# ZrrSkywalker/MonoDETR

Measured on NVIDIA H100. Metric: images/sec (1280x384, fwd+bwd), higher is better.
Workload: dtype f32 (BF16x3: error-compensated bf16 tensor-core products, fp32 accumulate)

## Files before the change

### monodetr_b200/csrc/conv_gemm.cu

```cuda
#include <cuda.h>
#include <cuda_runtime.h>
#include <stdint.h>
#include <stdlib.h>
#include <string.h>

#include "../../include/monodetr_b200.h"
#include "launch.cuh"
#include "tc_common.cuh"
#include "tma_host.cuh"

namespace {

using namespace mdb;

constexpr int BM = 128;
constexpr int BK = 32;
constexpr int kTileABytes = BM * 128;
constexpr int kChunkBytes = 32 * 128;
constexpr int kConsumerThreads = 256;
constexpr int kThreadsTC = kConsumerThreads + 32;
constexpr int kMaxTaps = 9;

struct TcParams {
    int tiles_x, tiles_y, tw, th, tb;
    int Ho, Wo;
    int out_sy, out_sx, out_oy, out_ox, out_H, out_W;
    int in_sy, in_sx;
    int ntaps, cblocks;
    int tap_dy[kMaxTaps], tap_dx[kMaxTaps], tap_w[kMaxTaps];
    int rtiles_x, rtiles_y, rtw, rth, n_img, red_per_split;
    int kb_per_slice, slice_stride;
    int total_tiles, n_tiles_n, n_tiles_m;
    int w_sy, w_sx, wg_taps, wg_kw, wg_pad;
    int Mo_rows;
    int No, ldo;
    int relu, atomic_out, round_out;
    int epi_tma, epi_load, half_x, half_y, half_b;
    const float* bias;
    const float* residual;
    const float* relu_mask;
    const float* rowscale;
    float* out;
};

template <bool MN>
__device__ __forceinline__ uint32_t raw_off(int row, int k) {
    if constexpr (MN) return (uint32_t)((row >> 5) * kChunkBytes + k * 128 + (((((row & 31) >> 2) ^ (k & 7))) << 4) + (row & 3) * 4);
    else return (uint32_t)(row * 128 + (((k >> 2) ^ (row & 7)) << 4) + (k & 3) * 4);
}

__device__ __forceinline__ float trunc_tf32(float x) { return __uint_as_float(__float_as_uint(x) & 0xFFFFE000u); }

template <int BN, int STAGES, int MODE, int PREC>
struct TcSmem {
    static constexpr bool kConvB = !(PREC == 2 && MODE == 0);
    static constexpr int kRing = STAGES * (kTileABytes + BN * 128);
    static constexpr int kStage = 2 * 64 * BN * 4;
    static constexpr int kConvBuf = kConvB ? (PREC == 1 ? 2 : 1) * BN * 128 : 0;
    static constexpr int kConv = 2 * kConvBuf;
    static constexpr int kFixed = kRing + kConv + 1024  + 256 ;
    static constexpr bool kTmaEpi = MODE == 0 && kFixed + kStage <= 227 * 1024;
    static constexpr int kBytes = kFixed + (kTmaEpi ? kStage : 0);
};

template <int BN, int STAGES, int MODE , bool B_MN, int PREC>
__global__ void __launch_bounds__(kThreadsTC, 1)
tc_conv_gemm_kernel(const __grid_constant__ CUtensorMap mapA, const __grid_constant__ CUtensorMap mapB,
                    const __grid_constant__ CUtensorMap mapO, const __grid_constant__ CUtensorMap mapR,
                    const __grid_constant__ TcParams p) {
    constexpr bool A_MN = (MODE == 1);
    static_assert(!(MODE == 1) || B_MN, "wgrad reads both operands MN-major");
    static_assert(BN == 64 || BN == 128, "tile width");
    constexpr bool BF_B = (PREC == 2 && MODE == 0);
    static_assert(!BF_B || !B_MN, "pre-split weights are K-major");
    constexpr bool CONVB = !BF_B;
    constexpr int kTileBBytes = BN * 128;
    constexpr int kRawBytes = kTileABytes + kTileBBytes;
    using SM = TcSmem<BN, STAGES, MODE, PREC>;
    constexpr int NACC = BN / 2;

    extern __shared__ __align__(1024) uint8_t smem[];
    uint8_t* stage_out = smem + STAGES * kRawBytes;
    uint8_t* bconv = stage_out + (SM::kTmaEpi ? SM::kStage : 0);
    uint64_t* full_bar = reinterpret_cast<uint64_t*>(bconv + SM::kConv);
    uint64_t* empty_bar = full_bar + STAGES;
    uint64_t* epi_bar = empty_bar + STAGES;

    const int warp = threadIdx.x >> 5;
    const int lane = threadIdx.x & 31;

    struct Tile { int n0, img, y0, x0, m0, red_begin, iters, tap, slice; };
    auto decode = [&](int tix) {
        Tile t;
        t.n0 = (tix % p.n_tiles_n) * BN;
        int r = tix / p.n_tiles_n;
        t.img = t.y0 = t.x0 = t.m0 = t.red_begin = t.tap = t.slice = 0;
        if constexpr (MODE == 0) {
            const int per_img = p.tiles_x * p.tiles_y;
            t.iters = p.ntaps * p.cblocks;
            if (p.kb_per_slice > 0) {
                t.slice = r / p.n_tiles_m;
                r -= t.slice * p.n_tiles_m;
                t.red_begin = t.slice * p.kb_per_slice;
                t.iters = max(0, min(t.iters, t.red_begin + p.kb_per_slice) - t.red_begin);
            }
            const int grp = r / per_img;
            t.img = grp * p.tb;
            r -= grp * per_img;
            t.y0 = (r / p.tiles_x) * p.th;
            t.x0 = (r % p.tiles_x) * p.tw;
        } else {
            t.m0 = (r % p.n_tiles_m) * BM;
            r /= p.n_tiles_m;
            t.tap = r % p.wg_taps;
            const int z = r / p.wg_taps;
            const int total_red = p.n_img * p.rtiles_x * p.rtiles_y;
            t.red_begin = z * p.red_per_split;
            t.iters = max(0, min(total_red, t.red_begin + p.red_per_split) - t.red_begin);
        }
        return t;
    };

    if (threadIdx.x == 0) {
        if (smem_u32(smem) & 1023u) __trap();
        tma_prefetch_desc(&mapA);
        tma_prefetch_desc(&mapB);
        if (SM::kTmaEpi && p.epi_tma) {
            tma_prefetch_desc(&mapO);
            if (p.epi_load) tma_prefetch_desc(&mapR);
        }
        for (int s = 0; s < STAGES; ++s) {
            mbar_init(&full_bar[s], 1);
            mbar_init(&empty_bar[s], kConsumerThreads / 32);
        }
        mbar_init(&epi_bar[0], 1);
        mbar_init(&epi_bar[1], 1);
        fence_mbar_init();
    }
    __syncthreads();
    asm volatile("griddepcontrol.wait;" ::: "memory");
    asm volatile("griddepcontrol.launch_dependents;" ::: "memory");

    if (warp == kConsumerThreads / 32) {
        if (elect_one()) {
            int git = 0;
            for (int tix = blockIdx.x; tix < p.total_tiles; tix += gridDim.x) {
                const Tile t = decode(tix);
                for (int it = 0; it < t.iters; ++it, ++git) {
                    const int s = git % STAGES;
                    const uint32_t ph = (git / STAGES) & 1;
                    mbar_wait(&empty_bar[s], ph ^ 1);
                    uint8_t* a_dst = smem + s * kRawBytes;
                    uint8_t* b_dst = a_dst + kTileABytes;
                    mbar_arrive_expect_tx(&full_bar[s], kRawBytes);
                    if constexpr (MODE == 0) {
                        const int kit = t.red_begin + it;
                        const int tap = kit / p.cblocks;
                        const int cb = kit - tap * p.cblocks;
                        tma_load_4d(a_dst, &mapA, &full_bar[s], cb * BK, t.x0 * p.in_sx + p.tap_dx[tap],
                                    t.y0 * p.in_sy + p.tap_dy[tap], t.img);
                        if constexpr (BF_B) {
                            tma_load_3d(b_dst, &mapB, &full_bar[s], cb * 64, t.n0, p.tap_w[tap]);
                        } else if constexpr (!B_MN) {
                            tma_load_3d(b_dst, &mapB, &full_bar[s], cb * BK, t.n0, p.tap_w[tap]);
                        } else {
#pragma unroll
                            for (int j = 0; j < BN / 32; ++j)
                                tma_load_3d(b_dst + j * kChunkBytes, &mapB, &full_bar[s], t.n0 + j * 32, cb * BK, p.tap_w[tap]);
                        }
                    } else {
                        int r = t.red_begin + it;
                        const int per_img = p.rtiles_x * p.rtiles_y;
                        const int ri = r / per_img;
                        r -= ri * per_img;
                        const int ry = (r / p.rtiles_x) * p.rth;
                        const int rx = (r % p.rtiles_x) * p.rtw;
#pragma unroll
                        for (int j = 0; j < BM / 32; ++j)
                            tma_load_4d(a_dst + j * kChunkBytes, &mapA, &full_bar[s], t.m0 + j * 32, rx, ry, ri);
#pragma unroll
                        for (int j = 0; j < BN / 32; ++j)
                            tma_load_4d(b_dst + j * kChunkBytes, &mapB, &full_bar[s], t.n0 + j * 32,
                                        rx * p.w_sx + (t.tap % p.wg_kw) - p.wg_pad, ry * p.w_sy + (t.tap / p.wg_kw) - p.wg_pad, ri);
                    }
                }
            }
        }
        return;
    }
    if (warp > kConsumerThreads / 32) return;

    const int wg = warp >> 2;
    const int g = lane >> 2, tig = lane & 3;
    const int r0 = wg * 64 + (warp & 3) * 16 + g;
    const int ctid = threadIdx.x;
    const bool epi_tma = SM::kTmaEpi && p.epi_tma;
    const bool leader = (ctid & 127) == 0;
    uint8_t* my_stage = stage_out + wg * (SM::kStage / 2);
    uint32_t epi_phase = 0;
    constexpr int KS = PREC == 2 ? 2 : 4;
    using Frag = uint32_t[KS][4];
    auto load_kblock = [&](int gi, int buf, Frag& hi, Frag& lo) {
        const int s = gi % STAGES;
        mbar_wait(&full_bar[s], (gi / STAGES) & 1);
        const uint8_t* a_raw = smem + s * kRawBytes;
        if constexpr (CONVB) {
            const uint8_t* b_raw = a_raw + kTileABytes;
            uint8_t* bc = bconv + buf * SM::kConvBuf;
            named_bar_sync(1, kConsumerThreads);
            if constexpr (PREC == 2) {
#pragma unroll
                for (int i = ctid; i < BN * 4; i += kConsumerThreads) {
                    const int n = i % BN, c = i / BN;
                    float x[8];
#pragma unroll
                    for (int e = 0; e < 8; ++e) x[e] = *reinterpret_cast<const float*>(b_raw + raw_off<B_MN>(n, 8 * c + e));
                    uint32_t hw[4], lw[4];
#pragma unroll
                    for (int e = 0; e < 4; ++e) {
                        const uint32_t h = pack_bf16x2(x[2 * e], x[2 * e + 1]);
                        hw[e] = h;
                        lw[e] = pack_bf16x2(x[2 * e] - __uint_as_float(h << 16), x[2 * e + 1] - __uint_as_float(h & 0xFFFF0000u));
                    }
                    uint8_t* brow = bc + n * 128;
                    *reinterpret_cast<uint4*>(brow + ((c ^ (n & 7)) << 4)) = make_uint4(hw[0], hw[1], hw[2], hw[3]);
                    *reinterpret_cast<uint4*>(brow + (((4 + c) ^ (n & 7)) << 4)) = make_uint4(lw[0], lw[1], lw[2], lw[3]);
                }
            } else {
#pragma unroll 4
                for (int i = ctid; i < BN * 8; i += kConsumerThreads) {
                    const int n = i % BN, c = i / BN;
                    float4 x;
                    if constexpr (B_MN) {
                        x.x = *reinterpret_cast<const float*>(b_raw + raw_off<true>(n, 4 * c));
                        x.y = *reinterpret_cast<const float*>(b_raw + raw_off<true>(n, 4 * c + 1));
                        x.z = *reinterpret_cast<const float*>(b_raw + raw_off<true>(n, 4 * c + 2));
                        x.w = *reinterpret_cast<const float*>(b_raw + raw_off<true>(n, 4 * c + 3));
                    } else {
                        x = *reinterpret_cast<const float4*>(b_raw + raw_off<false>(n, 4 * c));
                    }
                    const float4 h = make_float4(trunc_tf32(x.x), trunc_tf32(x.y), trunc_tf32(x.z), trunc_tf32(x.w));
                    const uint32_t off = n * 128 + ((c ^ (n & 7)) << 4);
                    *reinterpret_cast<float4*>(bc + off) = h;
                    if constexpr (PREC == 1)
                        *reinterpret_cast<float4*>(bc + kTileBBytes + off) = make_float4(x.x - h.x, x.y - h.y, x.z - h.z, x.w - h.w);
                }
            }
            fence_proxy_async_smem();
            named_bar_sync(1, kConsumerThreads);
        }
#pragma unroll
        for (int ks = 0; ks < KS; ++ks) {
#pragma unroll
            for (int f = 0; f < 4; ++f) {
                const int row = r0 + (f & 1) * 8;
                if constexpr (PREC == 2) {
                    const int k = ks * 16 + tig * 2 + (f >> 1) * 8;
                    float x0, x1;
                    if constexpr (A_MN) {
                        x0 = *reinterpret_cast<const float*>(a_raw + raw_off<true>(row, k));
                        x1 = *reinterpret_cast<const float*>(a_raw + raw_off<true>(row, k + 1));
                    } else {
                        const float2 v = *reinterpret_cast<const float2*>(a_raw + raw_off<false>(row, k));
                        x0 = v.x; x1 = v.y;
                    }
                    const uint32_t h = pack_bf16x2(x0, x1);
                    hi[ks][f] = h;
                    lo[ks][f] = pack_bf16x2(x0 - __uint_as_float(h << 16), x1 - __uint_as_float(h & 0xFFFF0000u));
                } else {
                    const int k = ks * 8 + tig + (f >> 1) * 4;
                    const float x = *reinterpret_cast<const float*>(a_raw + raw_off<A_MN>(row, k));
                    const float h = trunc_tf32(x);
                    hi[ks][f] = __float_as_uint(h);
                    lo[ks][f] = __float_as_uint(x - h);
                }
            }
        }
    };
    auto issue_kblock = [&](int gi, int buf, const Frag& hi, const Frag& lo, float (&acc)[NACC]) {
        const uint32_t b_addr = smem_u32(CONVB ? bconv + buf * SM::kConvBuf : smem + (gi % STAGES) * kRawBytes + kTileABytes);
        wgmma_fence();
#pragma unroll
        for (int ks = 0; ks < KS; ++ks) {
            const uint64_t bhi = make_wgmma_desc_sw128(b_addr + ks * 32);
            const uint64_t blo = make_wgmma_desc_sw128(b_addr + (PREC == 2 ? 64 : kTileBBytes) + ks * 32);
            if constexpr (PREC == 2) {
                if constexpr (BN == 128) {
                    wgmma_bf16_n128(acc, hi[ks], bhi, 1);
                    wgmma_bf16_n128(acc, lo[ks], bhi, 1);
                    wgmma_bf16_n128(acc, hi[ks], blo, 1);
                } else {
                    wgmma_bf16_n64(acc, hi[ks], bhi, 1);
                    wgmma_bf16_n64(acc, lo[ks], bhi, 1);
                    wgmma_bf16_n64(acc, hi[ks], blo, 1);
                }
            } else {
                if constexpr (BN == 128) wgmma_tf32_n128(acc, hi[ks], bhi, 1);
                else wgmma_tf32_n64(acc, hi[ks], bhi, 1);
                if constexpr (PREC == 1) {
                    if constexpr (BN == 128) {
                        wgmma_tf32_n128(acc, lo[ks], bhi, 1);
                        wgmma_tf32_n128(acc, hi[ks], blo, 1);
                    } else {
                        wgmma_tf32_n64(acc, lo[ks], bhi, 1);
                        wgmma_tf32_n64(acc, hi[ks], blo, 1);
                    }
                }
            }
        }
        wgmma_commit();
    };
    int git = 0;
    for (int tix = blockIdx.x; tix < p.total_tiles; tix += gridDim.x) {
        const Tile t = decode(tix);
        if (p.atomic_out && t.iters == 0) continue;
        const int c1 = t.x0 + wg * p.half_x, c2 = t.y0 + wg * p.half_y, c3 = t.img + wg * p.half_b, c4 = t.slice;
        if (epi_tma && p.epi_load && leader) {
            bulk_wait_read_all();
            mbar_arrive_expect_tx(&epi_bar[wg], SM::kStage / 2);
#pragma unroll
            for (int c = 0; c < BN / 32; ++c) tma_load_5d(my_stage + c * 8192, &mapR, &epi_bar[wg], t.n0 + 32 * c, c1, c2, c3, c4);
        }
        float acc[NACC];
#pragma unroll
        for (int i = 0; i < NACC; ++i) acc[i] = 0.f;
        if (t.iters > 0) {
            Frag ahi0, alo0, ahi1, alo1;
            auto step = [&](int it, const Frag& chi, const Frag& clo, Frag& nhi, Frag& nlo) {
                issue_kblock(git + it, it & 1, chi, clo, acc);
                wgmma_wait<1>();
                wgmma_fence_operands(nhi);
                wgmma_fence_operands(nlo);
                if (it > 0) {
                    __syncwarp();
                    if (lane == 0) mbar_arrive(&empty_bar[(git + it - 1) % STAGES]);
                }
                if (it + 1 < t.iters) load_kblock(git + it + 1, (it + 1) & 1, nhi, nlo);
            };
            load_kblock(git, 0, ahi0, alo0);
            for (int it = 0; it < t.iters; it += 2) {
                step(it, ahi0, alo0, ahi1, alo1);
                if (it + 1 < t.iters) step(it + 1, ahi1, alo1, ahi0, alo0);
            }
            wgmma_wait<0>();
            wgmma_fence_operands(acc);
            wgmma_fence_operands(ahi0);
            wgmma_fence_operands(alo0);
            wgmma_fence_operands(ahi1);
            wgmma_fence_operands(alo1);
            __syncwarp();
            if (lane == 0) mbar_arrive(&empty_bar[(git + t.iters - 1) % STAGES]);
            git += t.iters;
        }

        if (epi_tma) {
            if (p.bias) {
#pragma unroll
                for (int j = 0; j < BN / 8; ++j) {
                    const int n = t.n0 + j * 8 + tig * 2;
                    if (n >= p.No) continue;
                    const float b0 = p.bias[n], b1 = p.bias[n + 1];
                    acc[4 * j] += b0; acc[4 * j + 1] += b1; acc[4 * j + 2] += b0; acc[4 * j + 3] += b1;
                }
            }
            if (p.epi_load) {
                mbar_wait(&epi_bar[wg], epi_phase);
                epi_phase ^= 1;
            } else {
                if (leader) bulk_wait_read_all();
                named_bar_sync(2 + wg, 128);
            }
            constexpr int kMB = 8;
#pragma unroll
            for (int h = 0; h < 2; ++h) {
                const int row = r0 + h * 8, rr = row - 64 * wg;
                const float* gmask = nullptr;
                if (p.relu_mask && p.epi_load != 2) {
                    const int lyt = row / p.tw, lx = row - lyt * p.tw;
                    const int ib = lyt / p.th, ly = lyt - ib * p.th;
                    const int y = t.y0 + ly, x = t.x0 + lx, img = t.img + ib;
                    if ((y < p.Ho) && (x < p.Wo) && (img < p.n_img))
                        gmask = p.relu_mask + (size_t)((img * p.out_H + y * p.out_sy + p.out_oy) * p.out_W + x * p.out_sx + p.out_ox) * p.ldo;
                }
#pragma unroll
                for (int j0 = 0; j0 < BN / 8; j0 += kMB) {
                    float2 mv[kMB];
#pragma unroll
                    for (int u = 0; u < kMB; ++u) {
                        const int n = t.n0 + (j0 + u) * 8 + tig * 2;
                        mv[u] = (gmask && n < p.No) ? *reinterpret_cast<const float2*>(gmask + n) : make_float2(0.f, 0.f);
                    }
#pragma unroll
                    for (int u = 0; u < kMB; ++u) {
                        const int j = j0 + u, n = t.n0 + j * 8 + tig * 2;
                        if (n >= p.No) continue;
                        float2* sp = reinterpret_cast<float2*>(my_stage + (j >> 2) * 8192 + raw_off<false>(rr, (j & 3) * 8 + tig * 2));
                        float v[2] = {acc[4 * j + 2 * h], acc[4 * j + 2 * h + 1]};
                        if (p.epi_load == 1) { const float2 e = *sp; v[0] += e.x; v[1] += e.y; }
                        if (p.relu) { v[0] = fmaxf(v[0], 0.f); v[1] = fmaxf(v[1], 0.f); }
                        if (p.relu_mask) {
                            const float2 m = p.epi_load == 2 ? *sp : mv[u];
                            v[0] = m.x > 0.f ? v[0] : 0.f; v[1] = m.y > 0.f ? v[1] : 0.f;
                        }
                        if (p.round_out) { v[0] = round_tf32(v[0]); v[1] = round_tf32(v[1]); }
                        *sp = make_float2(v[0], v[1]);
                    }
                }
            }
            fence_proxy_async_smem();
            named_bar_sync(2 + wg, 128);
            if (leader) {
#pragma unroll
                for (int c = 0; c < BN / 32; ++c) tma_store_5d(&mapO, my_stage + c * 8192, t.n0 + 32 * c, c1, c2, c3, c4);
                bulk_commit();
            }
            continue;
        }
#pragma unroll
        for (int h = 0; h < 2; ++h) {
            const int row = r0 + h * 8;
            bool ok;
            size_t roff;
            float rsc = 1.f;
            if constexpr (MODE == 0) {
                const int lyt = row / p.tw, lx = row - lyt * p.tw;
                const int ib = lyt / p.th, ly = lyt - ib * p.th;
                const int y = t.y0 + ly, x = t.x0 + lx, img = t.img + ib;
                ok = (y < p.Ho) && (x < p.Wo) && (img < p.n_img);
                const int oy = y * p.out_sy + p.out_oy, ox = x * p.out_sx + p.out_ox;
                roff = (size_t)((img * p.out_H + oy) * p.out_W + ox) * p.ldo + (size_t)t.slice * p.slice_stride;
            } else {
                ok = (t.m0 + row) < p.Mo_rows;
                if (ok && p.rowscale) rsc = p.rowscale[t.m0 + row];
                roff = (size_t)(t.tap * p.Mo_rows + t.m0 + row) * p.ldo;
            }
            if (!ok) continue;
            const bool vec = !(p.ldo & 1);
#pragma unroll
            for (int j = 0; j < BN / 8; ++j) {
                const int n = t.n0 + j * 8 + tig * 2;
                if (n >= p.No) continue;
                float v[2] = {acc[4 * j + 2 * h] * rsc, acc[4 * j + 2 * h + 1] * rsc};
                const bool pair = vec && n + 1 < p.No;
                if (p.bias) { v[0] += p.bias[n]; if (pair) v[1] += p.bias[n + 1]; }
                if (p.residual) {
                    if (pair) { const float2 e = *reinterpret_cast<const float2*>(p.residual + roff + n); v[0] += e.x; v[1] += e.y; }
                    else v[0] += p.residual[roff + n];
                }
                if (p.relu) { v[0] = fmaxf(v[0], 0.f); v[1] = fmaxf(v[1], 0.f); }
                if (p.relu_mask) {
                    if (pair) {
                        const float2 m = *reinterpret_cast<const float2*>(p.relu_mask + roff + n);
                        v[0] = m.x > 0.f ? v[0] : 0.f; v[1] = m.y > 0.f ? v[1] : 0.f;
                    } else {
                        v[0] = p.relu_mask[roff + n] > 0.f ? v[0] : 0.f;
                    }
                }
                if (p.round_out) { v[0] = round_tf32(v[0]); v[1] = round_tf32(v[1]); }
                float* dst = p.out + roff + n;
                if (pair) {
                    if (p.atomic_out) red_add_v2_f32(dst, v[0], v[1]);
                    else *reinterpret_cast<float2*>(dst) = make_float2(v[0], v[1]);
                } else {
                    for (int e = 0; e < 2 && n + e < p.No; ++e) {
                        float x = e == 0 ? v[0] : acc[4 * j + 2 * h + 1] * rsc;
                        if (e == 1) {
                            if (p.bias) x += p.bias[n + 1];
                            if (p.residual) x += p.residual[roff + n + 1];
                            if (p.relu) x = fmaxf(x, 0.f);
                            if (p.relu_mask) x = p.relu_mask[roff + n + 1] > 0.f ? x : 0.f;
                            if (p.round_out) x = round_tf32(x);
                        }
                        if (p.atomic_out) atomicAdd(dst + e, x);
                        else dst[e] = x;
                    }
                }
            }
        }
    }
    if (epi_tma && leader) bulk_wait_all();
}

int g_precision = 2;

constexpr int kMaxDevices = 64;
struct DeviceState {
    float* ws = nullptr;
    size_t ws_bytes = 0;
};
DeviceState g_dev[kMaxDevices];

int current_device() {
    int dev = 0;
    if (cudaGetDevice(&dev) != cudaSuccess || dev < 0 || dev >= kMaxDevices) return 0;
    return dev;
}

template <int BN, int STAGES, int MODE, bool B_MN, int PREC>
int launch_tc(const CUtensorMap& a, const CUtensorMap& b, const CUtensorMap& o, const CUtensorMap& r, TcParams p, dim3 grid,
              cudaStream_t stream) {
    constexpr int smem = TcSmem<BN, STAGES, MODE, PREC>::kBytes;
    static_assert(smem <= 227 * 1024, "dynamic shared memory budget");
    if (!TcSmem<BN, STAGES, MODE, PREC>::kTmaEpi) p.epi_tma = p.epi_load = 0;
    auto kern = tc_conv_gemm_kernel<BN, STAGES, MODE, B_MN, PREC>;
    const cudaError_t e = set_max_dynamic_smem(kern, smem);
    if (e != cudaSuccess) return (int)e;
    p.n_tiles_n = (int)grid.x;
    p.n_tiles_m = (int)grid.y;
    p.total_tiles = (int)(grid.x * grid.y * grid.z);
    int ctas = num_sms();
    if (ctas > p.total_tiles) ctas = p.total_tiles;
    if (ctas < 1) return 0;
    static const bool pdl = getenv("MDB_NO_PDL") == nullptr;
    if (pdl) {
        cudaLaunchConfig_t cfg;
        memset(&cfg, 0, sizeof(cfg));
        cfg.gridDim = dim3((unsigned)ctas, 1, 1);
        cfg.blockDim = dim3((unsigned)kThreadsTC, 1, 1);
        cfg.dynamicSmemBytes = smem;
        cfg.stream = stream;
        cudaLaunchAttribute attr[1];
        attr[0].id = cudaLaunchAttributeProgrammaticStreamSerialization;
        attr[0].val.programmaticStreamSerializationAllowed = 1;
        cfg.attrs = attr;
        cfg.numAttrs = 1;
        return (int)cudaLaunchKernelEx(&cfg, kern, a, b, o, r, p);
    }
    kern<<<ctas, kThreadsTC, smem, stream>>>(a, b, o, r, p);
    return (int)cudaGetLastError();
}

__global__ void splitk_reduce_kernel(const float4* __restrict__ ws, const float4* __restrict__ bias, float4* __restrict__ y,
                                     long long n4, int N4, int slices, long long stride4) {
    for (long long i = blockIdx.x * (long long)blockDim.x + threadIdx.x; i < n4; i += (long long)gridDim.x * blockDim.x) {
        float4 a = bias ? bias[i % N4] : make_float4(0.f, 0.f, 0.f, 0.f);
        for (int z = 0; z < slices; ++z) {
            const float4 v = ws[z * stride4 + i];
            a.x += v.x; a.y += v.y; a.z += v.z; a.w += v.w;
        }
        y[i] = a;
    }
}

int splitk_workspace(size_t bytes, float** out) {
    DeviceState& d = g_dev[current_device()];
    if (bytes > d.ws_bytes || !d.ws) return MDB_EWORKSPACE;
    *out = d.ws;
    return 0;
}

void pick_tile(int W, int H, int n_pix, int* tw, int* th) {
    int best_tw = n_pix, best_waste = 1 << 30;
    for (int w = n_pix; w >= 1; w >>= 1) {
        const int h = n_pix / w;
        const int tx = (W + w - 1) / w, ty = (H + h - 1) / h;
        const int waste = tx * w * ty * h - W * H;
        if (waste < best_waste) { best_waste = waste; best_tw = w; }
    }
    *tw = best_tw;
    *th = n_pix / best_tw;
}

void pick_tile3(int W, int H, int B, int n_pix, int* tw, int* th, int* tb) {
    long long best = -1;
    *tw = n_pix; *th = 1; *tb = 1;
    for (int b = 1; b <= n_pix; b <<= 1)
        for (int w = n_pix / b; w >= 1; w >>= 1) {
            const int h = n_pix / b / w;
            if (b > 1 && b >= 2 * B) continue;
            const long long cov = (long long)((W + w - 1) / w) * w * ((H + h - 1) / h) * h * ((B + b - 1) / b) * b;
            if (best < 0 || cov < best) { best = cov; *tw = w; *th = h; *tb = b; }
        }
}

bool aligned16(const void* q) { return (reinterpret_cast<uintptr_t>(q) & 15u) == 0; }

int setup_epi_px(TcParams& p, CUtensorMap* mo, CUtensorMap* mr, size_t off, int Wc, int Hc, int B, uint64_t sx, uint64_t sy,
                 uint64_t sb, int slices) {
    p.epi_tma = p.epi_load = p.half_x = p.half_y = p.half_b = 0;
    if (p.No % 4 || p.ldo % 4 || !aligned16(p.out + off) || (p.residual && !aligned16(p.residual + off)) ||
        (p.relu_mask && !aligned16(p.relu_mask + off)))
        return 0;
    uint32_t box[5] = {32, (uint32_t)p.tw, (uint32_t)p.th, (uint32_t)p.tb, 1};
    if (p.tb > 1) p.half_b = box[3] = p.tb / 2;
    else if (p.th > 1) p.half_y = box[2] = p.th / 2;
    else p.half_x = box[1] = p.tw / 2;
    if (box[1] > 256 || box[2] > 256 || box[3] > 256) return 0;
    uint64_t dims[5] = {(uint64_t)p.No, (uint64_t)Wc, (uint64_t)Hc, (uint64_t)B, (uint64_t)slices};
    uint64_t str[5] = {1, sx, sy, sb, slices > 1 ? (uint64_t)p.slice_stride : sb * B};
    int rc = make_map(mo, p.out + off, 5, dims, str, box, nullptr);
    if (rc) return rc;
    const float* opnd = p.residual ? p.residual : p.relu_mask;
    if (opnd) {
        rc = make_map(mr, opnd + off, 5, dims, str, box, nullptr);
        if (rc) return rc;
        p.epi_load = p.residual ? 1 : 2;
    }
    p.epi_tma = 1;
    return 0;
}

int launch_fwd(const CUtensorMap& ma, const CUtensorMap& mb, const CUtensorMap& mo, const CUtensorMap& mr, const TcParams& p, dim3 grid, int bn, int precision, cudaStream_t stream) {
    if (precision == 2) return bn == 64 ? launch_tc<64, 6, 0, false, 2>(ma, mb, mo, mr, p, grid, stream) : launch_tc<128, 5, 0, false, 2>(ma, mb, mo, mr, p, grid, stream);
    if (precision == 1) return bn == 64 ? launch_tc<64, 5, 0, false, 1>(ma, mb, mo, mr, p, grid, stream) : launch_tc<128, 3, 0, false, 1>(ma, mb, mo, mr, p, grid, stream);
    return bn == 64 ? launch_tc<64, 6, 0, false, 0>(ma, mb, mo, mr, p, grid, stream) : launch_tc<128, 5, 0, false, 0>(ma, mb, mo, mr, p, grid, stream);
}

struct ConvGeom {
    int B, H, W, Cin, Cout, kh, kw, stride, pad, Ho, Wo;
};

// ... 236 lines not shown
    d.ws = static_cast<float*>(buf);
    d.ws_bytes = buf ? (size_t)bytes : 0;
    return 0;
}
int mdb_conv2d_dgrad_f32(const float* dy, const float* w_packed, const float* residual, const float* relu_mask,
                         float* dx, int B, int H, int W, int Cin, int Cout, int kh, int kw, int stride, int pad,
                         int flags, void* stream) {
    return conv_dgrad_impl(dy, w_packed, false, residual, relu_mask, dx, B, H, W, Cin, Cout, kh, kw, stride, pad, flags, stream);
}
int mdb_conv2d_dgrad_bf16x3(const float* dy, const void* w_split_t, const float* residual, const float* relu_mask,
                            float* dx, int B, int H, int W, int Cin, int Cout, int kh, int kw, int stride, int pad,
                            int flags, void* stream) {
    return conv_dgrad_impl(dy, w_split_t, true, residual, relu_mask, dx, B, H, W, Cin, Cout, kh, kw, stride, pad, flags, stream);
}

int mdb_conv2d_wgrad_f32(const float* dy, const float* x, const float* rowscale, float* dw_packed, int B, int H, int W,
                         int Cin, int Cout, int kh, int kw, int stride, int pad, int accumulate, void* stream_) {
    return mdb_conv2d_wgrad_bias_f32(dy, x, rowscale, dw_packed, nullptr, B, H, W, Cin, Cout, kh, kw, stride, pad, accumulate, stream_);
}

int mdb_conv2d_wgrad_bias_f32(const float* dy, const float* x, const float* rowscale, float* dw_packed, float* db, int B, int H,
                              int W, int Cin, int Cout, int kh, int kw, int stride, int pad, int accumulate, void* stream_) {
    ConvGeom g{B, H, W, Cin, Cout, kh, kw, stride, pad, (H + 2 * pad - kh) / stride + 1, (W + 2 * pad - kw) / stride + 1};
    int rc = check_geom(g);
    if (rc) return rc;
    if (!dy || !x || !dw_packed) return MDB_EINVAL;
    cudaStream_t stream = static_cast<cudaStream_t>(stream_);
    if (kh == 1 && stride == 1 && pad == 0) {
        W = B * H * W; H = 1; B = 1;
        g = ConvGeom{B, H, W, Cin, Cout, kh, kw, stride, pad, H, W};
    }
    const int taps = kh * kw;
    if (!accumulate) {
        cudaError_t e = cudaMemsetAsync(dw_packed, 0, sizeof(float) * (size_t)taps * Cout * Cin, stream);
        if (e != cudaSuccess) return (int)e;
    }
    if (db) {
        rc = mdb_colsum_f32(dy, db, (long long)B * g.Ho * g.Wo, Cout, accumulate, stream_);
        if (rc) return rc;
    }
    TcParams p;
    memset(&p, 0, sizeof(p));
    pick_tile(g.Wo, g.Ho, 32, &p.rtw, &p.rth);
    p.rtiles_x = (g.Wo + p.rtw - 1) / p.rtw;
    p.rtiles_y = (g.Ho + p.rth - 1) / p.rth;
    p.n_img = B;
    const int total_red = B * p.rtiles_x * p.rtiles_y;
    const int bn = 128;
    const int tiles = ((Cout + BM - 1) / BM) * ((Cin + bn - 1) / bn) * taps;
    const int sms = num_sms();
    int big = (2 * sms + tiles - 1) / tiles, small = sms / tiles;
    if (big > total_red / 24) big = total_red / 24;
    if (small > total_red / 8) small = total_red / 8;
    int splits = big > small ? big : small;
    if (splits < 1 || mdb_get_deterministic()) splits = 1;
    p.red_per_split = (total_red + splits - 1) / splits;
    splits = (total_red + p.red_per_split - 1) / p.red_per_split;
    p.w_sy = p.w_sx = stride;
    p.wg_taps = taps; p.wg_kw = kw; p.wg_pad = pad;
    p.Mo_rows = Cout; p.No = Cin; p.ldo = Cin; p.relu = 0; p.atomic_out = 1;
    p.bias = nullptr; p.residual = nullptr; p.relu_mask = nullptr; p.rowscale = rowscale;
    p.out = dw_packed;

    CUtensorMap ma, mb;
    {
        uint64_t dims[4] = {(uint64_t)Cout, (uint64_t)g.Wo, (uint64_t)g.Ho, (uint64_t)B};
        uint64_t str[4] = {1, (uint64_t)Cout, (uint64_t)g.Wo * Cout, (uint64_t)g.Ho * g.Wo * Cout};
        uint32_t box[4] = {32, (uint32_t)p.rtw, (uint32_t)p.rth, 1};
        rc = make_map(&ma, dy, 4, dims, str, box, nullptr);
        if (rc) return rc;
    }
    {
        uint64_t dims[4] = {(uint64_t)Cin, (uint64_t)W, (uint64_t)H, (uint64_t)B};
        uint64_t str[4] = {1, (uint64_t)Cin, (uint64_t)W * Cin, (uint64_t)H * W * Cin};
        uint32_t box[4] = {32, (uint32_t)(p.rtw * stride), (uint32_t)(p.rth * stride), 1};
        uint32_t es[4] = {1, (uint32_t)stride, (uint32_t)stride, 1};
        rc = make_map(&mb, x, 4, dims, str, box, es);
        if (rc) return rc;
    }
    CUtensorMap mo, mr;
    memset(&mo, 0, sizeof(mo));
    memset(&mr, 0, sizeof(mr));
    dim3 grid((Cin + bn - 1) / bn, (Cout + BM - 1) / BM, taps * splits);
    rc = g_precision == 2 ? launch_tc<128, 4, 1, true, 2>(ma, mb, mo, mr, p, grid, stream)
         : g_precision == 1 ? launch_tc<128, 4, 1, true, 1>(ma, mb, mo, mr, p, grid, stream)
                            : launch_tc<128, 5, 1, true, 0>(ma, mb, mo, mr, p, grid, stream);
    if (rc) return rc;
    return 0;
}

}
```

### monodetr_b200/csrc/tc_common.cuh

```cuda
#pragma once
#include <cuda.h>
#include <cuda_runtime.h>
#include <stdint.h>

namespace mdb {

__device__ __forceinline__ uint32_t smem_u32(const void* p) {
    return static_cast<uint32_t>(__cvta_generic_to_shared(p));
}

__device__ __forceinline__ bool elect_one() {
    uint32_t pred = 0;
    asm volatile(
        "{\n\t.reg .b32 rx;\n\t.reg .pred px;\n\t"
        "elect.sync rx|px, 0xffffffff;\n\t"
        "selp.b32 %0, 1, 0, px;\n\t}"
        : "=r"(pred));
    return pred != 0;
}

__device__ __forceinline__ void mbar_init(uint64_t* bar, uint32_t count) {
    asm volatile("mbarrier.init.shared::cta.b64 [%0], %1;" ::"r"(smem_u32(bar)), "r"(count) : "memory");
}
__device__ __forceinline__ void fence_mbar_init() {
// ... 26 lines not shown
    uint32_t spins = 0;
    uint64_t t0 = 0;
    while (!mbar_try_wait(bar, parity)) {
        if (++spins == 16384u) {
            spins = 0;
            mbar_slow_path(t0);
        }
    }
}

__device__ __forceinline__ void fence_proxy_async_smem() { asm volatile("fence.proxy.async.shared::cta;" ::: "memory"); }
__device__ __forceinline__ void named_bar_sync(int id, int count) { asm volatile("bar.sync %0, %1;" ::"r"(id), "r"(count) : "memory"); }

__device__ __forceinline__ void tma_prefetch_desc(const CUtensorMap* m) {
    asm volatile("prefetch.tensormap [%0];" ::"l"(reinterpret_cast<uint64_t>(m)) : "memory");
}
__device__ __forceinline__ void tma_load_2d(void* dst, const CUtensorMap* m, uint64_t* bar, int c0, int c1) {
    asm volatile(
        "cp.async.bulk.tensor.2d.shared::cluster.global.mbarrier::complete_tx::bytes [%0], [%1, {%3, %4}], [%2];" ::"r"(
            smem_u32(dst)),
        "l"(reinterpret_cast<uint64_t>(m)), "r"(smem_u32(bar)), "r"(c0), "r"(c1)
        : "memory");
}
__device__ __forceinline__ void tma_load_3d(void* dst, const CUtensorMap* m, uint64_t* bar, int c0, int c1, int c2) {
    asm volatile(
        "cp.async.bulk.tensor.3d.shared::cluster.global.mbarrier::complete_tx::bytes [%0], [%1, {%3, %4, %5}], [%2];" ::"r"(
            smem_u32(dst)),
        "l"(reinterpret_cast<uint64_t>(m)), "r"(smem_u32(bar)), "r"(c0), "r"(c1), "r"(c2)
        : "memory");
}
__device__ __forceinline__ void tma_load_4d(void* dst, const CUtensorMap* m, uint64_t* bar, int c0, int c1, int c2,
                                            int c3) {
    asm volatile(
        "cp.async.bulk.tensor.4d.shared::cluster.global.mbarrier::complete_tx::bytes [%0], [%1, {%3, %4, %5, %6}], "
        "[%2];" ::"r"(smem_u32(dst)),
        "l"(reinterpret_cast<uint64_t>(m)), "r"(smem_u32(bar)), "r"(c0), "r"(c1), "r"(c2), "r"(c3)
        : "memory");
}
__device__ __forceinline__ void tma_load_5d(void* dst, const CUtensorMap* m, uint64_t* bar, int c0, int c1, int c2,
                                            int c3, int c4) {
    asm volatile(
        "cp.async.bulk.tensor.5d.shared::cluster.global.mbarrier::complete_tx::bytes [%0], [%1, {%3, %4, %5, %6, %7}], "
        "[%2];" ::"r"(smem_u32(dst)),
        "l"(reinterpret_cast<uint64_t>(m)), "r"(smem_u32(bar)), "r"(c0), "r"(c1), "r"(c2), "r"(c3), "r"(c4)
        : "memory");
}
__device__ __forceinline__ void tma_store_5d(const CUtensorMap* m, const void* src, int c0, int c1, int c2, int c3, int c4) {
    asm volatile("cp.async.bulk.tensor.5d.global.shared::cta.bulk_group [%0, {%2, %3, %4, %5, %6}], [%1];"
                 ::"l"(reinterpret_cast<uint64_t>(m)), "r"(smem_u32(src)), "r"(c0), "r"(c1), "r"(c2), "r"(c3), "r"(c4)
                 : "memory");
}
__device__ __forceinline__ void bulk_commit() { asm volatile("cp.async.bulk.commit_group;" ::: "memory"); }
__device__ __forceinline__ void bulk_wait_read_all() { asm volatile("cp.async.bulk.wait_group.read 0;" ::: "memory"); }
__device__ __forceinline__ void bulk_wait_all() { asm volatile("cp.async.bulk.wait_group 0;" ::: "memory"); }

__device__ __forceinline__ void wgmma_fence() { asm volatile("wgmma.fence.sync.aligned;" ::: "memory"); }
__device__ __forceinline__ void wgmma_commit() { asm volatile("wgmma.commit_group.sync.aligned;" ::: "memory"); }
__device__ __forceinline__ void wgmma_wait_all() { asm volatile("wgmma.wait_group.sync.aligned 0;" ::: "memory"); }
template <int N>
__device__ __forceinline__ void wgmma_wait() { asm volatile("wgmma.wait_group.sync.aligned %0;" ::"n"(N) : "memory"); }
template <int N>
__device__ __forceinline__ void wgmma_fence_operands(float (&d)[N]) {
#pragma unroll
    for (int i = 0; i < N; ++i) asm volatile("" : "+f"(d[i])::"memory");
}
template <int M, int N>
__device__ __forceinline__ void wgmma_fence_operands(uint32_t (&a)[M][N]) {
#pragma unroll
    for (int i = 0; i < M; ++i)
#pragma unroll
        for (int j = 0; j < N; ++j) asm volatile("" : "+r"(a[i][j])::"memory");
}
__device__ __forceinline__ void wgmma_bf16_n64(float (&d)[32], const uint32_t (&a)[4], uint64_t bdesc, int scale_d) {
    asm volatile(
        "{\n\t.reg .pred p;\n\t"
        "setp.ne.b32 p, %37, 0;\n\t"
        "wgmma.mma_async.sync.aligned.m64n64k16.f32.bf16.bf16 "
        "{%0, %1, %2, %3, %4, %5, %6, %7, %8, %9, %10, %11, %12, %13, %14, %15, "
        "%16, %17, %18, %19, %20, %21, %22, %23, %24, %25, %26, %27, %28, %29, %30, %31"
        "}, {%32, %33, %34, %35}, %36, p, 1, 1, 0;\n\t}"
        : "+f"(d[0]), "+f"(d[1]), "+f"(d[2]), "+f"(d[3]), "+f"(d[4]), "+f"(d[5]), "+f"(d[6]), "+f"(d[7]), "+f"(d[8]), "+f"(d[9]), "+f"(d[10]), "+f"(d[11]), "+f"(d[12]), "+f"(d[13]), "+f"(d[14]), "+f"(d[15]), "+f"(d[16]), "+f"(d[17]), "+f"(d[18]), "+f"(d[19]), "+f"(d[20]), "+f"(d[21]), "+f"(d[22]), "+f"(d[23]), "+f"(d[24]), "+f"(d[25]), "+f"(d[26]), "+f"(d[27]), "+f"(d[28]), "+f"(d[29]), "+f"(d[30]), "+f"(d[31])
        : "r"(a[0]), "r"(a[1]), "r"(a[2]), "r"(a[3]), "l"(bdesc), "r"(scale_d));
}
__device__ __forceinline__ void wgmma_bf16_n128(float (&d)[64], const uint32_t (&a)[4], uint64_t bdesc, int scale_d) {
    asm volatile(
        "{\n\t.reg .pred p;\n\t"
        "setp.ne.b32 p, %69, 0;\n\t"
        "wgmma.mma_async.sync.aligned.m64n128k16.f32.bf16.bf16 "
        "{%0, %1, %2, %3, %4, %5, %6, %7, %8, %9, %10, %11, %12, %13, %14, %15, "
        "%16, %17, %18, %19, %20, %21, %22, %23, %24, %25, %26, %27, %28, %29, %30, %31, "
        "%32, %33, %34, %35, %36, %37, %38, %39, %40, %41, %42, %43, %44, %45, %46, %47, "
        "%48, %49, %50, %51, %52, %53, %54, %55, %56, %57, %58, %59, %60, %61, %62, %63"
        "}, {%64, %65, %66, %67}, %68, p, 1, 1, 0;\n\t}"
        : "+f"(d[0]), "+f"(d[1]), "+f"(d[2]), "+f"(d[3]), "+f"(d[4]), "+f"(d[5]), "+f"(d[6]), "+f"(d[7]), "+f"(d[8]), "+f"(d[9]), "+f"(d[10]), "+f"(d[11]), "+f"(d[12]), "+f"(d[13]), "+f"(d[14]), "+f"(d[15]), "+f"(d[16]), "+f"(d[17]), "+f"(d[18]), "+f"(d[19]), "+f"(d[20]), "+f"(d[21]), "+f"(d[22]), "+f"(d[23]), "+f"(d[24]), "+f"(d[25]), "+f"(d[26]), "+f"(d[27]), "+f"(d[28]), "+f"(d[29]), "+f"(d[30]), "+f"(d[31]), "+f"(d[32]), "+f"(d[33]), "+f"(d[34]), "+f"(d[35]), "+f"(d[36]), "+f"(d[37]), "+f"(d[38]), "+f"(d[39]), "+f"(d[40]), "+f"(d[41]), "+f"(d[42]), "+f"(d[43]), "+f"(d[44]), "+f"(d[45]), "+f"(d[46]), "+f"(d[47]), "+f"(d[48]), "+f"(d[49]), "+f"(d[50]), "+f"(d[51]), "+f"(d[52]), "+f"(d[53]), "+f"(d[54]), "+f"(d[55]), "+f"(d[56]), "+f"(d[57]), "+f"(d[58]), "+f"(d[59]), "+f"(d[60]), "+f"(d[61]), "+f"(d[62]), "+f"(d[63])
        : "r"(a[0]), "r"(a[1]), "r"(a[2]), "r"(a[3]), "l"(bdesc), "r"(scale_d));
}
__device__ __forceinline__ void wgmma_tf32_n32(float (&d)[16], const uint32_t (&a)[4], uint64_t bdesc, int scale_d) {
    asm volatile(
        "{\n\t.reg .pred p;\n\t"
        "setp.ne.b32 p, %21, 0;\n\t"
        "wgmma.mma_async.sync.aligned.m64n32k8.f32.tf32.tf32 "
        "{%0, %1, %2, %3, %4, %5, %6, %7, %8, %9, %10, %11, %12, %13, %14, %15"
        "}, {%16, %17, %18, %19}, %20, p, 1, 1;\n\t}"
        : "+f"(d[0]), "+f"(d[1]), "+f"(d[2]), "+f"(d[3]), "+f"(d[4]), "+f"(d[5]), "+f"(d[6]), "+f"(d[7]), "+f"(d[8]), "+f"(d[9]), "+f"(d[10]), "+f"(d[11]), "+f"(d[12]), "+f"(d[13]), "+f"(d[14]), "+f"(d[15])
        : "r"(a[0]), "r"(a[1]), "r"(a[2]), "r"(a[3]), "l"(bdesc), "r"(scale_d));
}

__device__ __forceinline__ void wgmma_tf32_n64(float (&d)[32], const uint32_t (&a)[4], uint64_t bdesc, int scale_d) {
    asm volatile(
        "{\n\t.reg .pred p;\n\t"
        "setp.ne.b32 p, %37, 0;\n\t"
        "wgmma.mma_async.sync.aligned.m64n64k8.f32.tf32.tf32 "
        "{%0, %1, %2, %3, %4, %5, %6, %7, %8, %9, %10, %11, %12, %13, %14, %15, "
        "%16, %17, %18, %19, %20, %21, %22, %23, %24, %25, %26, %27, %28, %29, %30, %31"
        "}, {%32, %33, %34, %35}, %36, p, 1, 1;\n\t}"
        : "+f"(d[0]), "+f"(d[1]), "+f"(d[2]), "+f"(d[3]), "+f"(d[4]), "+f"(d[5]), "+f"(d[6]), "+f"(d[7]), "+f"(d[8]), "+f"(d[9]), "+f"(d[10]), "+f"(d[11]), "+f"(d[12]), "+f"(d[13]), "+f"(d[14]), "+f"(d[15]), "+f"(d[16]), "+f"(d[17]), "+f"(d[18]), "+f"(d[19]), "+f"(d[20]), "+f"(d[21]), "+f"(d[22]), "+f"(d[23]), "+f"(d[24]), "+f"(d[25]), "+f"(d[26]), "+f"(d[27]), "+f"(d[28]), "+f"(d[29]), "+f"(d[30]), "+f"(d[31])
        : "r"(a[0]), "r"(a[1]), "r"(a[2]), "r"(a[3]), "l"(bdesc), "r"(scale_d));
}
__device__ __forceinline__ void wgmma_tf32_n128(float (&d)[64], const uint32_t (&a)[4], uint64_t bdesc, int scale_d) {
    asm volatile(
        "{\n\t.reg .pred p;\n\t"
        "setp.ne.b32 p, %69, 0;\n\t"
        "wgmma.mma_async.sync.aligned.m64n128k8.f32.tf32.tf32 "
        "{%0, %1, %2, %3, %4, %5, %6, %7, %8, %9, %10, %11, %12, %13, %14, %15, "
        "%16, %17, %18, %19, %20, %21, %22, %23, %24, %25, %26, %27, %28, %29, %30, %31, "
        "%32, %33, %34, %35, %36, %37, %38, %39, %40, %41, %42, %43, %44, %45, %46, %47, "
        "%48, %49, %50, %51, %52, %53, %54, %55, %56, %57, %58, %59, %60, %61, %62, %63"
        "}, {%64, %65, %66, %67}, %68, p, 1, 1;\n\t}"
        : "+f"(d[0]), "+f"(d[1]), "+f"(d[2]), "+f"(d[3]), "+f"(d[4]), "+f"(d[5]), "+f"(d[6]), "+f"(d[7]), "+f"(d[8]), "+f"(d[9]), "+f"(d[10]), "+f"(d[11]), "+f"(d[12]), "+f"(d[13]), "+f"(d[14]), "+f"(d[15]), "+f"(d[16]), "+f"(d[17]), "+f"(d[18]), "+f"(d[19]), "+f"(d[20]), "+f"(d[21]), "+f"(d[22]), "+f"(d[23]), "+f"(d[24]), "+f"(d[25]), "+f"(d[26]), "+f"(d[27]), "+f"(d[28]), "+f"(d[29]), "+f"(d[30]), "+f"(d[31]), "+f"(d[32]), "+f"(d[33]), "+f"(d[34]), "+f"(d[35]), "+f"(d[36]), "+f"(d[37]), "+f"(d[38]), "+f"(d[39]), "+f"(d[40]), "+f"(d[41]), "+f"(d[42]), "+f"(d[43]), "+f"(d[44]), "+f"(d[45]), "+f"(d[46]), "+f"(d[47]), "+f"(d[48]), "+f"(d[49]), "+f"(d[50]), "+f"(d[51]), "+f"(d[52]), "+f"(d[53]), "+f"(d[54]), "+f"(d[55]), "+f"(d[56]), "+f"(d[57]), "+f"(d[58]), "+f"(d[59]), "+f"(d[60]), "+f"(d[61]), "+f"(d[62]), "+f"(d[63])
        : "r"(a[0]), "r"(a[1]), "r"(a[2]), "r"(a[3]), "l"(bdesc), "r"(scale_d));
}


__device__ __forceinline__ uint32_t pack_bf16x2(float lo, float hi) {
    uint32_t r;
    asm("cvt.rn.bf16x2.f32 %0, %1, %2;" : "=r"(r) : "f"(hi), "f"(lo));
    return r;
}

__device__ __forceinline__ uint64_t make_wgmma_desc_sw128(uint32_t smem_addr) {
    return (uint64_t)((smem_addr & 0x3FFFFu) >> 4) | ((uint64_t)1 << 16) | ((uint64_t)(1024 >> 4) << 32) | ((uint64_t)1 << 62);
}

__device__ __forceinline__ float round_tf32(float v) {
    uint32_t r;
    asm("cvt.rna.tf32.f32 %0, %1;" : "=r"(r) : "f"(v));
    return __uint_as_float(r);
}

__device__ __forceinline__ void red_add_v4_f32(float* addr, float a, float b, float c, float d) {
    asm volatile("red.global.add.v4.f32 [%0], {%1, %2, %3, %4};" ::"l"(addr), "f"(a), "f"(b), "f"(c), "f"(d) : "memory");
}

__device__ __forceinline__ void red_add_v2_f32(float* addr, float a, float b) {
    asm volatile("red.global.add.v2.f32 [%0], {%1, %2};" ::"l"(addr), "f"(a), "f"(b) : "memory");
}

}
```

Baseline: 143.4.

## Add dedicated converter warpgroup for bf16x3 wgrad B-operand splitting

For the weight-gradient GEMM in split-bf16 precision mode, a separate 128-thread converter warpgroup now splits raw fp32 B tiles into hi/lo bf16 halves in an MN-major swizzled layout. It uses a triple-buffered operand ring with its own full/empty mbarriers, and the consumers issue transposed-B bf16 wgmma straight from it. This takes the conversion off the consumer warpgroups' critical path. Registers are rebalanced with setmaxnreg, and the wgrad pipeline depth goes from 4 to 5 stages, which adds shared memory use and synchronisation complexity.

```diff
diff --git a/monodetr_b200/csrc/conv_gemm.cu b/monodetr_b200/csrc/conv_gemm.cu
--- a/monodetr_b200/csrc/conv_gemm.cu
+++ b/monodetr_b200/csrc/conv_gemm.cu
@@ -20,6 +20,13 @@
 constexpr int kConsumerThreads = 256;
 constexpr int kThreadsTC = kConsumerThreads + 32;
 constexpr int kMaxTaps = 9;
+
+template <int MODE, int PREC>
+constexpr bool kConvWG = MODE == 1 && PREC == 2;
+template <int MODE, int PREC>
+constexpr int kThreads = kConvWG<MODE, PREC> ? kConsumerThreads + 256 : kThreadsTC;
+constexpr int kRegConsumer = 184, kRegConverter = 96, kRegProducer = 40;
+static_assert(2 * 128 * kRegConsumer + 128 * (kRegConverter + kRegProducer) <= 65536, "register file");
 
 struct TcParams {
     int tiles_x, tiles_y, tw, th, tb;
@@ -57,14 +64,15 @@
     static constexpr int kRing = STAGES * (kTileABytes + BN * 128);
     static constexpr int kStage = 2 * 64 * BN * 4;
     static constexpr int kConvBuf = kConvB ? (PREC == 1 ? 2 : 1) * BN * 128 : 0;
-    static constexpr int kConv = 2 * kConvBuf;
+    static constexpr int kOpBufs = kConvWG<MODE, PREC> ? 3 : 2;
+    static constexpr int kConv = kOpBufs * kConvBuf;
     static constexpr int kFixed = kRing + kConv + 1024  + 256 ;
     static constexpr bool kTmaEpi = MODE == 0 && kFixed + kStage <= 227 * 1024;
     static constexpr int kBytes = kFixed + (kTmaEpi ? kStage : 0);
 };
 
 template <int BN, int STAGES, int MODE , bool B_MN, int PREC>
-__global__ void __launch_bounds__(kThreadsTC, 1)
+__global__ void __launch_bounds__(kThreads<MODE, PREC>, 1)
 tc_conv_gemm_kernel(const __grid_constant__ CUtensorMap mapA, const __grid_constant__ CUtensorMap mapB,
                     const __grid_constant__ CUtensorMap mapO, const __grid_constant__ CUtensorMap mapR,
                     const __grid_constant__ TcParams p) {
@@ -73,7 +81,9 @@
     static_assert(BN == 64 || BN == 128, "tile width");
     constexpr bool BF_B = (PREC == 2 && MODE == 0);
     static_assert(!BF_B || !B_MN, "pre-split weights are K-major");
-    constexpr bool CONVB = !BF_B;
+    constexpr bool CONV_WG = kConvWG<MODE, PREC>;
+    static_assert(!CONV_WG || BN == 128, "converter item mapping");
+    constexpr bool CONVB = !BF_B && !CONV_WG;
     constexpr int kTileBBytes = BN * 128;
     constexpr int kRawBytes = kTileABytes + kTileBBytes;
     using SM = TcSmem<BN, STAGES, MODE, PREC>;
@@ -85,6 +95,8 @@
     uint64_t* full_bar = reinterpret_cast<uint64_t*>(bconv + SM::kConv);
     uint64_t* empty_bar = full_bar + STAGES;
     uint64_t* epi_bar = empty_bar + STAGES;
+    uint64_t* op_full = epi_bar + 2;
+    uint64_t* op_empty = op_full + SM::kOpBufs;
 
     const int warp = threadIdx.x >> 5;
     const int lane = threadIdx.x & 31;
@@ -131,18 +143,60 @@
         }
         for (int s = 0; s < STAGES; ++s) {
             mbar_init(&full_bar[s], 1);
-            mbar_init(&empty_bar[s], kConsumerThreads / 32);
+            mbar_init(&empty_bar[s], kConsumerThreads / 32 + (CONV_WG ? 4 : 0));
         }
         mbar_init(&epi_bar[0], 1);
         mbar_init(&epi_bar[1], 1);
+        if constexpr (CONV_WG) {
+            for (int o = 0; o < SM::kOpBufs; ++o) {
+                mbar_init(&op_full[o], 128);
+                mbar_init(&op_empty[o], kConsumerThreads / 32);
+            }
+        }
         fence_mbar_init();
     }
     __syncthreads();
     asm volatile("griddepcontrol.wait;" ::: "memory");
     asm volatile("griddepcontrol.launch_dependents;" ::: "memory");
 
-    if (warp == kConsumerThreads / 32) {
-        if (elect_one()) {
+    if (CONV_WG && warp >= kConsumerThreads / 32 + 4) {
+        if constexpr (CONV_WG) setmaxnreg_dec<kRegConverter>();
+        const int cw = warp - (kConsumerThreads / 32 + 4);
+        const int pc = lane & 7, jl = (lane >> 3) & 1, kl = lane >> 4;
+        constexpr int kHalf = BN * 64;
+        int git = 0;
+        for (int tix = blockIdx.x; tix < p.total_tiles; tix += gridDim.x) {
+            const Tile t = decode(tix);
+            for (int it = 0; it < t.iters; ++it, ++git) {
+                const int s = git % STAGES, o = git % SM::kOpBufs;
+                mbar_wait(&full_bar[s], (git / STAGES) & 1);
+                mbar_wait(&op_empty[o], ((git / SM::kOpBufs) & 1) ^ 1);
+                const uint8_t* b_raw = smem + s * kRawBytes + kTileABytes;
+                uint8_t* bc = bconv + o * SM::kConvBuf;
+#pragma unroll
+                for (int u = 0; u < BN / 16; ++u) {
+                    const int k = kl + 2 * cw + 8 * (u >> 1), j = jl + 2 * (u & 1);
+                    const int q = pc ^ (k & 7);
+                    const float4 x = *reinterpret_cast<const float4*>(b_raw + j * kChunkBytes + k * 128 + pc * 16);
+                    const uint32_t h0 = pack_bf16x2(x.x, x.y), h1 = pack_bf16x2(x.z, x.w);
+                    const uint32_t l0 = pack_bf16x2(x.x - __uint_as_float(h0 << 16), x.y - __uint_as_float(h0 & 0xFFFF0000u));
+                    const uint32_t l1 = pack_bf16x2(x.z - __uint_as_float(h1 << 16), x.w - __uint_as_float(h1 & 0xFFFF0000u));
+                    const uint32_t off = (k >> 3) * 2048 + (j >> 1) * 1024 + (k & 7) * 128 +
+                                         (((4 * (j & 1) + (q >> 1)) ^ (k & 7)) << 4) + (q & 1) * 8;
+                    *reinterpret_cast<uint2*>(bc + off) = make_uint2(h0, h1);
+                    *reinterpret_cast<uint2*>(bc + kHalf + off) = make_uint2(l0, l1);
+                }
+                fence_proxy_async_smem();
+                mbar_arrive(&op_full[o]);
+                __syncwarp();
+                if (lane == 0) mbar_arrive(&empty_bar[s]);
+            }
+        }
+        return;
+    }
+    if (warp >= kConsumerThreads / 32) {
+        if constexpr (CONV_WG) setmaxnreg_dec<kRegProducer>();
+        if (warp == kConsumerThreads / 32 && elect_one()) {
             int git = 0;
             for (int tix = blockIdx.x; tix < p.total_tiles; tix += gridDim.x) {
                 const Tile t = decode(tix);
@@ -188,7 +242,7 @@
         }
         return;
     }
-    if (warp > kConsumerThreads / 32) return;
+    if constexpr (CONV_WG) setmaxnreg_inc<kRegConsumer>();
 
     const int wg = warp >> 2;
     const int g = lane >> 2, tig = lane & 3;
@@ -278,6 +332,22 @@
         }
     };
     auto issue_kblock = [&](int gi, int buf, const Frag& hi, const Frag& lo, float (&acc)[NACC]) {
+        if constexpr (CONV_WG) {
+            const int o = gi % SM::kOpBufs;
+            mbar_wait(&op_full[o], (gi / SM::kOpBufs) & 1);
+            const uint32_t b_addr = smem_u32(bconv + o * SM::kConvBuf);
+            wgmma_fence();
+#pragma unroll
+            for (int ks = 0; ks < KS; ++ks) {
+                const uint64_t bhi = make_wgmma_desc_sw128_mn(b_addr + ks * 4096, 1024, 2048);
+                const uint64_t blo = make_wgmma_desc_sw128_mn(b_addr + BN * 64 + ks * 4096, 1024, 2048);
+                wgmma_bf16_n128<1>(acc, hi[ks], bhi, 1);
+                wgmma_bf16_n128<1>(acc, lo[ks], bhi, 1);
+                wgmma_bf16_n128<1>(acc, hi[ks], blo, 1);
+            }
+            wgmma_commit();
+            return;
+        }
         const uint32_t b_addr = smem_u32(CONVB ? bconv + buf * SM::kConvBuf : smem + (gi % STAGES) * kRawBytes + kTileABytes);
         wgmma_fence();
 #pragma unroll
@@ -333,7 +403,10 @@
                 wgmma_fence_operands(nlo);
                 if (it > 0) {
                     __syncwarp();
-                    if (lane == 0) mbar_arrive(&empty_bar[(git + it - 1) % STAGES]);
+                    if (lane == 0) {
+                        mbar_arrive(&empty_bar[(git + it - 1) % STAGES]);
+                        if constexpr (CONV_WG) mbar_arrive(&op_empty[(git + it - 1) % SM::kOpBufs]);
+                    }
                 }
                 if (it + 1 < t.iters) load_kblock(git + it + 1, (it + 1) & 1, nhi, nlo);
             };
@@ -349,7 +422,10 @@
             wgmma_fence_operands(ahi1);
             wgmma_fence_operands(alo1);
             __syncwarp();
-            if (lane == 0) mbar_arrive(&empty_bar[(git + t.iters - 1) % STAGES]);
+            if (lane == 0) {
+                mbar_arrive(&empty_bar[(git + t.iters - 1) % STAGES]);
+                if constexpr (CONV_WG) mbar_arrive(&op_empty[(git + t.iters - 1) % SM::kOpBufs]);
+            }
             git += t.iters;
         }
 
@@ -516,7 +592,7 @@
         cudaLaunchConfig_t cfg;
         memset(&cfg, 0, sizeof(cfg));
         cfg.gridDim = dim3((unsigned)ctas, 1, 1);
-        cfg.blockDim = dim3((unsigned)kThreadsTC, 1, 1);
+        cfg.blockDim = dim3((unsigned)kThreads<MODE, PREC>, 1, 1);
         cfg.dynamicSmemBytes = smem;
         cfg.stream = stream;
         cudaLaunchAttribute attr[1];
@@ -526,7 +602,7 @@
         cfg.numAttrs = 1;
         return (int)cudaLaunchKernelEx(&cfg, kern, a, b, o, r, p);
     }
-    kern<<<ctas, kThreadsTC, smem, stream>>>(a, b, o, r, p);
+    kern<<<ctas, kThreads<MODE, PREC>, smem, stream>>>(a, b, o, r, p);
     return (int)cudaGetLastError();
 }
 
@@ -929,7 +1005,7 @@
     memset(&mo, 0, sizeof(mo));
     memset(&mr, 0, sizeof(mr));
     dim3 grid((Cin + bn - 1) / bn, (Cout + BM - 1) / BM, taps * splits);
-    rc = g_precision == 2 ? launch_tc<128, 4, 1, true, 2>(ma, mb, mo, mr, p, grid, stream)
+    rc = g_precision == 2 ? launch_tc<128, 5, 1, true, 2>(ma, mb, mo, mr, p, grid, stream)
          : g_precision == 1 ? launch_tc<128, 4, 1, true, 1>(ma, mb, mo, mr, p, grid, stream)
                             : launch_tc<128, 5, 1, true, 0>(ma, mb, mo, mr, p, grid, stream);
     if (rc) return rc;
diff --git a/monodetr_b200/csrc/tc_common.cuh b/monodetr_b200/csrc/tc_common.cuh
--- a/monodetr_b200/csrc/tc_common.cuh
+++ b/monodetr_b200/csrc/tc_common.cuh
@@ -132,6 +132,7 @@
         : "+f"(d[0]), "+f"(d[1]), "+f"(d[2]), "+f"(d[3]), "+f"(d[4]), "+f"(d[5]), "+f"(d[6]), "+f"(d[7]), "+f"(d[8]), "+f"(d[9]), "+f"(d[10]), "+f"(d[11]), "+f"(d[12]), "+f"(d[13]), "+f"(d[14]), "+f"(d[15]), "+f"(d[16]), "+f"(d[17]), "+f"(d[18]), "+f"(d[19]), "+f"(d[20]), "+f"(d[21]), "+f"(d[22]), "+f"(d[23]), "+f"(d[24]), "+f"(d[25]), "+f"(d[26]), "+f"(d[27]), "+f"(d[28]), "+f"(d[29]), "+f"(d[30]), "+f"(d[31])
         : "r"(a[0]), "r"(a[1]), "r"(a[2]), "r"(a[3]), "l"(bdesc), "r"(scale_d));
 }
+template <int TRANS_B = 0>
 __device__ __forceinline__ void wgmma_bf16_n128(float (&d)[64], const uint32_t (&a)[4], uint64_t bdesc, int scale_d) {
     asm volatile(
         "{\n\t.reg .pred p;\n\t"
@@ -141,9 +142,9 @@
         "%16, %17, %18, %19, %20, %21, %22, %23, %24, %25, %26, %27, %28, %29, %30, %31, "
         "%32, %33, %34, %35, %36, %37, %38, %39, %40, %41, %42, %43, %44, %45, %46, %47, "
         "%48, %49, %50, %51, %52, %53, %54, %55, %56, %57, %58, %59, %60, %61, %62, %63"
-        "}, {%64, %65, %66, %67}, %68, p, 1, 1, 0;\n\t}"
+        "}, {%64, %65, %66, %67}, %68, p, 1, 1, %70;\n\t}"
         : "+f"(d[0]), "+f"(d[1]), "+f"(d[2]), "+f"(d[3]), "+f"(d[4]), "+f"(d[5]), "+f"(d[6]), "+f"(d[7]), "+f"(d[8]), "+f"(d[9]), "+f"(d[10]), "+f"(d[11]), "+f"(d[12]), "+f"(d[13]), "+f"(d[14]), "+f"(d[15]), "+f"(d[16]), "+f"(d[17]), "+f"(d[18]), "+f"(d[19]), "+f"(d[20]), "+f"(d[21]), "+f"(d[22]), "+f"(d[23]), "+f"(d[24]), "+f"(d[25]), "+f"(d[26]), "+f"(d[27]), "+f"(d[28]), "+f"(d[29]), "+f"(d[30]), "+f"(d[31]), "+f"(d[32]), "+f"(d[33]), "+f"(d[34]), "+f"(d[35]), "+f"(d[36]), "+f"(d[37]), "+f"(d[38]), "+f"(d[39]), "+f"(d[40]), "+f"(d[41]), "+f"(d[42]), "+f"(d[43]), "+f"(d[44]), "+f"(d[45]), "+f"(d[46]), "+f"(d[47]), "+f"(d[48]), "+f"(d[49]), "+f"(d[50]), "+f"(d[51]), "+f"(d[52]), "+f"(d[53]), "+f"(d[54]), "+f"(d[55]), "+f"(d[56]), "+f"(d[57]), "+f"(d[58]), "+f"(d[59]), "+f"(d[60]), "+f"(d[61]), "+f"(d[62]), "+f"(d[63])
-        : "r"(a[0]), "r"(a[1]), "r"(a[2]), "r"(a[3]), "l"(bdesc), "r"(scale_d));
+        : "r"(a[0]), "r"(a[1]), "r"(a[2]), "r"(a[3]), "l"(bdesc), "r"(scale_d), "n"(TRANS_B));
 }
 __device__ __forceinline__ void wgmma_tf32_n32(float (&d)[16], const uint32_t (&a)[4], uint64_t bdesc, int scale_d) {
     asm volatile(
@@ -191,6 +192,14 @@
 __device__ __forceinline__ uint64_t make_wgmma_desc_sw128(uint32_t smem_addr) {
     return (uint64_t)((smem_addr & 0x3FFFFu) >> 4) | ((uint64_t)1 << 16) | ((uint64_t)(1024 >> 4) << 32) | ((uint64_t)1 << 62);
 }
+__device__ __forceinline__ uint64_t make_wgmma_desc_sw128_mn(uint32_t smem_addr, uint32_t lbo, uint32_t sbo) {
+    return (uint64_t)((smem_addr & 0x3FFFFu) >> 4) | ((uint64_t)(lbo >> 4) << 16) | ((uint64_t)(sbo >> 4) << 32) | ((uint64_t)1 << 62);
+}
+
+template <int N>
+__device__ __forceinline__ void setmaxnreg_inc() { asm volatile("setmaxnreg.inc.sync.aligned.u32 %0;" ::"n"(N)); }
+template <int N>
+__device__ __forceinline__ void setmaxnreg_dec() { asm volatile("setmaxnreg.dec.sync.aligned.u32 %0;" ::"n"(N)); }
 
 __device__ __forceinline__ float round_tf32(float v) {
     uint32_t r;
```

New measurement: 146.8, median of 6. 2.4% higher.
